# itz-sayak/C-Users-Sayakdutta-Self-Supervised-Arbitrary-Scale-Point-Cloud-Upsampling-via-SNN

Measured on AMD Instinct MI355X. Metric: upsampled query-points/sec (kNN + fn fwd + rotate + fd fwd + displace), 4x scale, M=48 T=4, higher is better.
Workload: dtype f32 (GEMMs as 3 x f16 MFMA with f32 accumulation; outer kNN f64); 1 GPU; synthetic sphere N=5000 (seed 0), B=4096 grid queries per GPU per step, M=48, T=4, fn k=[24,18,12] emb 640, fd k=32 scales [8,16,32,48] emb 768, conditioned-random weights seed 0, in-patch kNN recomputed every batch; cloud_points=5000, neighbours=48, outer_knn=f64 brute force, parallelism=query shards x1

## Files before the change

c-users-sayakdutta-self-supervised-arbitrary-scale-point-cloud-upsampling-via-snn_amd/_lib.py:

```python
import ctypes
import os
from ctypes import POINTER, c_char_p, c_double, c_float, c_int, c_int32, c_int64, c_void_p

_HERE = os.path.dirname(os.path.abspath(__file__))
LIB_PATH = os.environ.get("SAPCU_LIB_PATH") or os.path.join(_HERE, "csrc", "libsapcu_hip.so")
EXACT_LIB_PATH = os.path.join(_HERE, "csrc", "libsapcu_hip_exact.so")

FN_TAPS = ("stem", "block1", "block2", "block3", "pooled", "enc", "logits")
FD_TAPS = ("fused0", "spikes", "knn", "pooled", "enc", "x0")
KIND_FN, KIND_FD = 0, 1
ABI_VERSION = 2


class SapcuLibraryError(RuntimeError):
    """The HIP library is absent or unloadable (never silently replaced by a CPU path)."""


class SapcuError(RuntimeError):
    """A C entry point returned a non-zero status: args = (code, text)."""


_SIGNATURES = {
    "sapcu_abi_version": (c_int, []),
    "sapcu_last_error": (c_char_p, []),
# ... 64 lines not shown
_FD_TRAIN_SIGNATURES = {
    "sapcu_fd_neuron_step_forward": (c_int, [c_void_p, c_int64, c_int, c_int] + [c_void_p] * 6 + [c_void_p] * 3 + [c_void_p] + [c_void_p] * 5 +
                                     [c_void_p]),
    "sapcu_fd_neuron_step_workspace_bytes": (c_int64, [c_int64, c_int]),
    "sapcu_fd_neuron_step_backward": (c_int, [c_void_p, c_void_p, c_int64, c_int, c_int] + [c_void_p] * 4 + [c_void_p] * 3 + [c_void_p] * 5 +
                                      [c_void_p, c_int64, c_void_p]),
    "sapcu_fd_edge_feature_forward": (c_int, [c_void_p, c_int, c_void_p, c_int64, c_int, c_int, c_int, c_int, c_void_p, c_void_p, c_void_p]),
    "sapcu_fd_edge_feature_backward": (c_int, [c_void_p, c_void_p, c_int64, c_int, c_int, c_int, c_int, c_void_p, c_int, c_void_p, c_void_p]),
    "sapcu_fd_bn_stats_workspace_bytes": (c_int64, [c_int64, c_int]),
    "sapcu_fd_bn_stats": (c_int, [c_void_p, c_int64, c_int, c_float, c_void_p, c_void_p, c_void_p, c_void_p, c_int64, c_void_p]),
    "sapcu_fd_bn_lrelu_max_forward": (c_int, [c_void_p, c_int64, c_int, c_int] + [c_void_p] * 4 + [c_void_p, c_void_p, c_void_p]),
    "sapcu_fd_bn_lrelu_max_backward": (c_int, [c_void_p, c_void_p, c_void_p, c_int64, c_int, c_int] + [c_void_p] * 4 + [c_void_p, c_void_p]),
}
FD_TRAIN_EXPORTS = tuple(_FD_TRAIN_SIGNATURES)

_FD_EDGECONV_SIGNATURES = {
    "sapcu_fd_edgeconv_stats_workspace_bytes": (c_int64, [c_int64, c_int, c_int, c_int]),
    "sapcu_fd_edgeconv_stats": (c_int, [c_void_p, c_void_p, c_int64, c_int, c_int, c_int, c_float] + [c_void_p] * 4 + [c_void_p, c_int64, c_void_p]),
    "sapcu_fd_edgeconv_max_forward": (c_int, [c_void_p, c_void_p, c_int64, c_int, c_int, c_int] + [c_void_p] * 4 + [c_void_p, c_void_p, c_void_p]),
    "sapcu_fd_edgeconv_backward_workspace_bytes": (c_int64, [c_int64, c_int, c_int, c_int]),
    "sapcu_fd_edgeconv_backward": (c_int, [c_void_p] * 4 + [c_int64, c_int, c_int, c_int] + [c_void_p] * 4 + [c_void_p] * 4 +
                                   [c_void_p, c_int64, c_void_p]),
}
FD_EDGECONV_EXPORTS = tuple(_FD_EDGECONV_SIGNATURES)

_TRAIN_STEP_SIGNATURES = {
    "sapcu_multi_select": (c_int, [c_void_p, c_void_p, c_void_p, c_void_p, c_int, c_int, c_void_p]),
}
TRAIN_STEP_EXPORTS = tuple(_TRAIN_STEP_SIGNATURES)

_METRICS_SIGNATURES = {
    "sapcu_nn_cross_workspace_bytes": (c_int64, [c_int64, c_int64]),
    "sapcu_nn_cross_grid_f64": (c_int, [c_void_p, c_int64, c_void_p, c_int64, c_double, c_void_p, c_void_p, c_void_p, c_int64,
                                        POINTER(c_int64), c_void_p]),
}
METRICS_EXPORTS = tuple(_METRICS_SIGNATURES)

_DATA_SIGNATURES = {
    "sapcu_train_patches_workspace_bytes": (c_int64, [c_int64]),
    "sapcu_train_patches_f32": (c_int, [c_void_p, c_int64, c_int, c_void_p, c_int, c_void_p, c_void_p, c_int64, c_void_p, c_void_p, c_void_p,
                                        c_void_p, c_int, c_int] + [c_void_p] * 7 + [c_void_p, c_int64, c_void_p]),
}
DATA_EXPORTS = tuple(_DATA_SIGNATURES)

_MESH_SIGNATURES = {
    "sapcu_point_mesh_workspace_bytes": (c_int64, [c_int64, c_int64, c_int64]),
    "sapcu_point_mesh_f64": (c_int, [c_void_p, c_int64, c_void_p, c_int64, c_void_p, c_int64, c_double, c_void_p, c_void_p, c_void_p,
                                     c_void_p, c_int64, POINTER(c_int64), c_void_p]),
}
MESH_EXPORTS = tuple(_MESH_SIGNATURES)

_INTERNAL_SIGNATURES = {
    "sapcu_internal_fold_affine_host": (c_int, [c_void_p, c_void_p, c_void_p, c_void_p, c_int, c_int, c_void_p, c_void_p]),
    "sapcu_internal_point_mesh_tuned": (c_int, [c_void_p, c_int64, c_void_p, c_int64, c_void_p, c_int64, c_double, c_double, c_int, c_int, c_void_p,
                                                c_void_p, c_void_p, c_void_p, c_int64, POINTER(c_int64), c_void_p]),
}
_lib = None


def load(path=None):
    global _lib
    if _lib is not None and path is None:
        return _lib
    p = path or LIB_PATH
    if not os.path.exists(p):
        raise SapcuLibraryError(
            "HIP library not built: %s is missing. Run `make -C %s` (needs hipcc, gfx950). "
            "There is no CPU fallback." % (p, os.path.dirname(p)))
    try:
        lib = ctypes.CDLL(p)
    except OSError as e:
        raise SapcuLibraryError("cannot load %s: %s" % (p, e)) from e
    for name, (res, args) in list(_SIGNATURES.items()) + list(_SEEDS_SIGNATURES.items()) + list(_FD_TRAIN_SIGNATURES.items()) + \
            list(_FD_EDGECONV_SIGNATURES.items()) + list(_TRAIN_STEP_SIGNATURES.items()) + list(_METRICS_SIGNATURES.items()) + \
            list(_DATA_SIGNATURES.items()) + list(_MESH_SIGNATURES.items()) + list(_INTERNAL_SIGNATURES.items()):
        try:
            fn = getattr(lib, name)
        except AttributeError as e:
            raise SapcuLibraryError("%s does not export %s" % (p, name)) from e
        fn.restype = res
        fn.argtypes = args
    if lib.sapcu_abi_version() != ABI_VERSION:
        raise SapcuLibraryError("ABI version mismatch: library %d, binding %d" % (lib.sapcu_abi_version(), ABI_VERSION))
    if path is None:
        _lib = lib
    return lib


def check(rc):
    if rc != 0:
        text = load().sapcu_last_error()
        raise SapcuError(int(rc), text.decode("utf-8", "replace") if text else "")


def ptr(t):
    return None if t is None else c_void_p(t.data_ptr())


def current_stream():
    import torch
    return c_void_p(torch.cuda.current_stream().cuda_stream)
```

c-users-sayakdutta-self-supervised-arbitrary-scale-point-cloud-upsampling-via-snn_amd/csrc/common.h:

```cpp
#pragma once
#include <hip/hip_runtime.h>
#include <stdint.h>
#include <stdio.h>
#include <string.h>
#include "../../include/sapcu.h"

namespace sapcu {

void set_error(const char* fmt, ...);

#define SAPCU_CHECK_ARG(cond, ...)                      \
    do {                                                \
        if (!(cond)) {                                  \
            ::sapcu::set_error(__VA_ARGS__);            \
            return SAPCU_ERR_ARG;                       \
        }                                               \
    } while (0)

#define SAPCU_CHECK_HIP(expr)                                                            \
    do {                                                                                 \
        hipError_t _e = (expr);                                                          \
        if (_e != hipSuccess) {                                                          \
            ::sapcu::set_error("%s failed: %s (%s:%d)", #expr, hipGetErrorString(_e),    \
                               __FILE__, __LINE__);                                      \
// ... 382 lines not shown
    const double s = sqrt(d);
    const double r = __fma_rn(-s, s, d);
    return __fma_rn(r, __ddiv_rn(0.5, s), s);
}

__device__ __forceinline__ float gelu_erf(float x) {
    return 0.5f * x * (1.0f + erff(x * 0.70710678118654752440f));
}
__device__ __forceinline__ float lrelu02(float x) { return x >= 0.f ? x : 0.2f * x; }
__device__ __forceinline__ unsigned float_max_key(float x) {
    const unsigned b = __float_as_uint(x);
    return (b & 0x80000000u) ? ~b : (b | 0x80000000u);
}
__device__ __forceinline__ float float_from_max_key(unsigned k) { return __uint_as_float((k & 0x80000000u) ? (k & 0x7fffffffu) : ~k); }

enum GemmEpi { EPI_BIAS = 0, EPI_LIF = 1, EPI_GELU = 2, EPI_RESID = 3, EPI_LRELU = 4, EPI_RESID_GELU = 5, EPI_LIF_ATTN = 6,
               EPI_LRELU_MAX = 7,
               EPI_LIF_MAX = 8 };

struct GemmArgs {
    const float* a;
    int64_t r;
    int k, lda;
    const float* w;
    int n;
    const float* bias;
    float* c;
    int ldc;
    int epi;
    const float* lif;
    int lif_T;
    const float* resid;
    int ldr;
    float* c2;
    const float* q;
    const float* kf;
    int ldq;
    const int2* tab;
    const _Float16* w16_hi;
    const _Float16* w16_lo;
    int* ovf;
    int a_split, c_split, c2_split;
    unsigned* max_keys;
    int max_m;
    float* max_out;
};
int launch_gemm(const GemmArgs& g, hipStream_t st);
int launch_gemm_sf16(const GemmArgs& g, hipStream_t st);
int launch_gemm_sf16_ring(const GemmArgs& g, hipStream_t st);
int launch_gemm_sf16_bt(const GemmArgs& g, hipStream_t st);
bool gemm_sf16_bt_ok(const GemmArgs& g);
bool gemm_shortk_ok(const GemmArgs& g);
int launch_gemm_shortk(const GemmArgs& g, hipStream_t st);
int launch_gemm_split_rows(const GemmArgs& g, hipStream_t st, bool allow_bt = true);
int launch_split_weights(const float* w, int64_t count, void* hi, void* lo, int* ovf, hipStream_t st);

int launch_knn_outer(const double* cloud, int64_t n, const double* q, int64_t b, int k, int64_t* idx,
                     double* dist, float* patch, hipStream_t st);
int launch_gather_rotate(const double* cloud, int64_t n, const double* q, int64_t b, const int64_t* idx,
                         int k, const float* normals, float* patch, hipStream_t st);
int launch_displace(const double* q, const float* nrm, const float* d, int64_t b, double* out, hipStream_t st);

size_t fps_workspace_bytes(int npoint);
int zero_count(int* p, hipStream_t st);
int launch_fps(const float* xyz, int64_t n, int npoint, int start, int64_t* out, void* ws, hipStream_t st);
int fps_failed(const void* ws, int npoint, int* flag);

}
```

c-users-sayakdutta-self-supervised-arbitrary-scale-point-cloud-upsampling-via-snn_amd/csrc/gemm_epi.h:

```cpp
#pragma once
#include "common.h"

namespace sapcu {

typedef float f32x16 __attribute__((ext_vector_type(16)));

typedef _Float16 epi_half8 __attribute__((ext_vector_type(8)));
typedef float epi_f32x4 __attribute__((ext_vector_type(4)));
__device__ __forceinline__ f32x16 mfma_32x32x16_f16(epi_half8 a, epi_half8 b, f32x16 c) {
#ifdef SAPCU_TIMING_MFMA16
    epi_f32x4 q0 = {c[0], c[1], c[2], c[3]}, q1 = {c[8], c[9], c[10], c[11]};
    q0 = __builtin_amdgcn_mfma_f32_16x16x32_f16(a, b, q0, 0, 0, 0);
    q1 = __builtin_amdgcn_mfma_f32_16x16x32_f16(a, b, q1, 0, 0, 0);
    c[0] = q0[0]; c[1] = q0[1]; c[2] = q0[2]; c[3] = q0[3];
    c[8] = q1[0]; c[9] = q1[1]; c[10] = q1[2]; c[11] = q1[3];
    return c;
#else
    return __builtin_amdgcn_mfma_f32_32x32x16_f16(a, b, c, 0, 0, 0);
#endif
}

__device__ __forceinline__ float4 ld4(const float* p) { return *reinterpret_cast<const float4*>(p); }

__device__ __forceinline__ void lds_barrier() { asm volatile("s_waitcnt lgkmcnt(0)\n\ts_barrier" ::: "memory"); }
// ... 98 lines not shown
    if (EPI == EPI_LIF || EPI == EPI_LIF_ATTN) {
        const int cc = valid ? col : 0;
        c.decay = ld4_cols<VEC>(g.lif, cc, g.n);
        c.adapt = ld4_cols<VEC>(g.lif + g.n, cc, g.n);
        c.rdecay = ld4_cols<VEC>(g.lif + 2 * (int64_t)g.n, cc, g.n);
        c.theta0 = ld4_cols<VEC>(g.lif + 3 * (int64_t)g.n, cc, g.n);
    }
    return c;
}

__device__ __forceinline__ void clamp_col_params4(const ColParams4& c, NeuronP2 (&np)[2]) {
    np[0].decay = f32x2{clampf(c.decay.x, 0.1f, 0.99f), clampf(c.decay.y, 0.1f, 0.99f)};
    np[1].decay = f32x2{clampf(c.decay.z, 0.1f, 0.99f), clampf(c.decay.w, 0.1f, 0.99f)};
    np[0].adapt = f32x2{clampf(c.adapt.x, 0.001f, 0.1f), clampf(c.adapt.y, 0.001f, 0.1f)};
    np[1].adapt = f32x2{clampf(c.adapt.z, 0.001f, 0.1f), clampf(c.adapt.w, 0.001f, 0.1f)};
    np[0].rdecay = f32x2{clampf(c.rdecay.x, 0.1f, 0.95f), clampf(c.rdecay.y, 0.1f, 0.95f)};
    np[1].rdecay = f32x2{clampf(c.rdecay.z, 0.1f, 0.95f), clampf(c.rdecay.w, 0.1f, 0.95f)};
    np[0].theta0 = f32x2{c.theta0.x, c.theta0.y};
    np[1].theta0 = f32x2{c.theta0.z, c.theta0.w};
}

typedef _Float16 half4 __attribute__((ext_vector_type(4)));

template <bool VEC>
__device__ __forceinline__ void store_f32x4(float* base, int64_t row, int ld, int col, int n, const float (&v)[4]) {
    if (VEC) {
        *reinterpret_cast<float4*>(base + row * ld + col) = make_float4(v[0], v[1], v[2], v[3]);
    } else {
#pragma unroll
        for (int u = 0; u < 4; ++u)
            if (col + u < n) base[row * ld + col + u] = v[u];
    }
}

template <bool VEC>
__device__ __forceinline__ void store_split4(float* base, int64_t row, int ld, int col, int n, const float (&v)[4]) {
    if (!VEC) {
#pragma unroll
        for (int u = 0; u < 4; ++u)
            if (col + u < n) store_split(base, row, ld, col + u, v[u]);
        return;
    }
    _Float16* rp = reinterpret_cast<_Float16*>(base + row * ld);
    half4 hi, lo;
#pragma unroll
    for (int u = 0; u < 4; ++u) {
        hi[u] = (_Float16)v[u];
        lo[u] = (_Float16)(v[u] - (float)hi[u]);
    }
    *reinterpret_cast<half4*>(rp + split_hi_index(ld, col)) = hi;
    *reinterpret_cast<half4*>(rp + split_lo_index(ld, col)) = lo;
}

template <int EPI, bool VEC>
__device__ __forceinline__ void epilogue_row4_compute(const GemmArgs& g, const float4 acc, int64_t row, int col,
                                                      const ColParams4& cp, float (&v)[4]) {
    v[0] = __fmaf_rn(acc.x, 0.0625f, cp.bias.x);
    v[1] = __fmaf_rn(acc.y, 0.0625f, cp.bias.y);
    v[2] = __fmaf_rn(acc.z, 0.0625f, cp.bias.z);
    v[3] = __fmaf_rn(acc.w, 0.0625f, cp.bias.w);
    float4 res = make_float4(0.f, 0.f, 0.f, 0.f);
    if (EPI == EPI_RESID || EPI == EPI_RESID_GELU) res = ld4_cols<VEC>(g.resid + row * g.ldr, col, g.n);
    if (EPI == EPI_LIF || EPI == EPI_LIF_ATTN) {
        f32x2 pv[2] = {f32x2{v[0], v[1]}, f32x2{v[2], v[3]}};
        NeuronP2 np[2];
        clamp_col_params4(cp, np);
        lif_selfloop_pairs<2>(pv, np, g.lif_T);
        v[0] = pv[0].x; v[1] = pv[0].y; v[2] = pv[1].x; v[3] = pv[1].y;
    }
    const float rs[4] = {res.x, res.y, res.z, res.w};
#pragma unroll
    for (int u = 0; u < 4; ++u) {
        if (EPI == EPI_GELU) v[u] = gelu_erf(v[u]);
        if (EPI == EPI_LRELU) v[u] = lrelu02(v[u]);
        if (EPI == EPI_RESID) v[u] = __fadd_rn(v[u], rs[u]);
        if (EPI == EPI_RESID_GELU) v[u] = gelu_erf(__fadd_rn(v[u], rs[u]));
    }
}

template <int EPI, bool VEC>
__device__ __forceinline__ void epilogue_row4_store(const GemmArgs& g, const float (&v)[4], int64_t row, int col,
                                                    const float4 q, const float4 kf) {
    float ai[4] = {0.f, 0.f, 0.f, 0.f};
    if (EPI == EPI_LIF_ATTN) {
        ai[0] = __fadd_rn(__fsub_rn(q.x, kf.x), v[0]);
        ai[1] = __fadd_rn(__fsub_rn(q.y, kf.y), v[1]);
        ai[2] = __fadd_rn(__fsub_rn(q.z, kf.z), v[2]);
        ai[3] = __fadd_rn(__fsub_rn(q.w, kf.w), v[3]);
        asm volatile("" : "+v"(ai[0]), "+v"(ai[1]), "+v"(ai[2]), "+v"(ai[3])::"memory");
    }
    if (g.c_split) {
        store_split4<VEC>(g.c, row, g.ldc, col, g.n, v);
        if (EPI != EPI_LIF && EPI != EPI_LIF_ATTN && g.ovf) {
            float big = 0.f;
#pragma unroll
            for (int u = 0; u < 4; ++u)
                if (VEC || col + u < g.n) big = fmaxf(big, fabsf(v[u]));
            const bool nan = (VEC || col < g.n) && !(v[0] == v[0] && v[1] == v[1] && v[2] == v[2] && v[3] == v[3]);
            if (!(big < 65504.0f) || nan) atomicAdd(g.ovf, 1);
        }
    } else {
        store_f32x4<VEC>(g.c, row, g.ldc, col, g.n, v);
    }
    if (EPI == EPI_LIF_ATTN) {
        if (g.c2_split) store_split4<VEC>(g.c2, row, g.ldc, col, g.n, ai);
        else store_f32x4<VEC>(g.c2, row, g.ldc, col, g.n, ai);
    }
}

template <int EPI>
__device__ __forceinline__ void epilogue_group4(const GemmArgs& g, const float (&acc)[4], int64_t row, int col,
                                                float bias, const NeuronP& np, const float (&q)[4],
                                                const float (&kf)[4]) {
    epilogue_group<EPI, 4>(g, acc, row, col, bias, np, q, kf);
}

}
```

c-users-sayakdutta-self-supervised-arbitrary-scale-point-cloud-upsampling-via-snn_amd/csrc/model.hip:

```cpp
#include <stdarg.h>
#include <stdlib.h>

#include <new>
#include <vector>

#include "common.h"
#include "ops.h"

namespace sapcu {

static thread_local char g_err[512] = "";

void set_error(const char* fmt, ...) {
    va_list ap;
    va_start(ap, fmt);
    vsnprintf(g_err, sizeof(g_err), fmt, ap);
    va_end(ap);
}

enum FnSlot {
    FN_STEM_W = 0, FN_STEM_B, FN_STEM_LIF,
    FN_BLK0 = 3,
    FN_FINAL_W = FN_BLK0 + 63, FN_FINAL_B, FN_FINAL_LIF,
    FN_FCOUT_W, FN_FCOUT_B,
// ... 5 lines not shown
    B_FC1_W = 0, B_FC1_B, B_SNN1,
    B_QKV_W, B_QKV_B, B_QKV_LIF,
    B_DELTA_W, B_DELTA_B, B_DELTA_LIF,
    B_DELTA2_W, B_DELTA2_B, B_DELTA2_LIF,
    B_GAMMA_W, B_GAMMA_B, B_GAMMA_LIF,
    B_GAMMA2_W, B_GAMMA2_B,
    B_OUT_W, B_OUT_B,
    B_FC2_W, B_FC2_B,
    B_SLOTS
};
static_assert(B_SLOTS == 21, "fn block slot count");
static_assert(FN_SLOTS == 81, "fn slot count");

enum FdSlot {
    FD_E0_W = 0, FD_E0_B,
    FD_FUSE_W, FD_FUSE_B, FD_SNN0,
    FD_EDGE1_W, FD_EDGE1_SHIFT, FD_SNN1,
    FD_EDGE2_W, FD_EDGE2_SHIFT, FD_SNN2,
    FD_EDGE3_W, FD_EDGE3_SHIFT, FD_SNN3,
    FD_MSC_W, FD_MSC_B,
    FD_TI_W, FD_SNNFC,
    FD_FCIN_W, FD_FCIN_B,
    FD_R0_FC0_W, FD_R0_FC0_B, FD_R0_FC4_W, FD_R0_FC4_B, FD_R0_PROJ_W, FD_R0_PROJ_B,
    FD_R1_FC0_W, FD_R1_FC0_B, FD_R1_FC4_W, FD_R1_FC4_B, FD_R1_PROJ_W, FD_R1_PROJ_B,
    FD_QKV_W, FD_QKV_B,
    FD_WO_T, FD_BO, FD_LN_W, FD_LN_B, FD_WH_T, FD_BH, FD_WD, FD_BD,
    FD_SLOTS
};
static_assert(FD_SLOTS == 42, "fd slot count");

}

struct sapcu_model {
    int kind = 0;
    int kv[3] = {0, 0, 0};
    int k = 0, nscale = 0;
    int ks[8] = {0, 0, 0, 0, 0, 0, 0, 0};
    int32_t* ks_dev = nullptr;
    int* gate_dev = nullptr;
    bool sf16 = true;
    void* w16_hi = nullptr;
    void* w16_lo = nullptr;
    void* chain_w = nullptr;
    int* ovf_dev = nullptr;
    int emb = 0, T = 0, heads = 0;
    int64_t chunk = 0;
    int64_t ws_budget = 0;
    bool opt_bt = true;
    bool opt_chain = true;
    bool opt_chain_wide = false;
    bool opt_chain_fill = true;
    bool opt_chain_trim = true;
    bool opt_shortk = true;
    bool opt_fn_maxfuse = true;
    bool opt_fn_fold_out = true;
    bool opt_fd_maxfuse = true;
    bool opt_fd_split = true;
    bool opt_fd_fused = true;
    bool opt_fd_x0 = true;
    void* fde_w = nullptr;
    int64_t fde_off[5] = {0, 0, 0, 0, 0};
    float* fde_nprm = nullptr;
    float* blob = nullptr;
    int64_t blob_floats = 0;
    int64_t fold_w[3] = {0, 0, 0}, fold_b[3] = {0, 0, 0};
    std::vector<int64_t> dir;
    const float* p(int slot) const { return blob + dir[slot]; }
};

namespace sapcu {

static inline int64_t imax(int64_t a, int64_t b) { return a > b ? a : b; }
static inline int imin(int a, int b) { return a < b ? a : b; }

static bool split_rows_gemm_on_big_tile(const GemmArgs& g, bool allow_bt) { return allow_bt && gemm_sf16_bt_ok(g); }

int launch_gemm_split_rows(const GemmArgs& g, hipStream_t st, bool allow_bt) {
    if (split_rows_gemm_on_big_tile(g, allow_bt)) return launch_gemm_sf16_bt(g, st);
    return launch_gemm_sf16_ring(g, st);
}

static void fold_affine_f64(const float* w1, const float* b1, const float* w2, const float* b2, int d, int n, float* w_fold,
                            float* b_fold) {
    std::vector<double> acc((size_t)d);
    for (int i = 0; i < n; ++i) {
        for (int k = 0; k < d; ++k) acc[k] = 0.0;
        double bs = 0.0;
        for (int j = 0; j < d; ++j) {
            const double a = (double)w2[(int64_t)i * d + j];
            const float* row = w1 + (int64_t)j * d;
            for (int k = 0; k < d; ++k) acc[k] += a * (double)row[k];
            bs += a * (double)b1[j];
        }
        for (int k = 0; k < d; ++k) w_fold[(int64_t)i * d + k] = (float)acc[k];
        b_fold[i] = (float)(bs + (double)b2[i]);
    }
}

static bool env_is(const char* name, const char* value) {
    const char* e = getenv(name);
    return e && strcmp(e, value) == 0;
}

static void read_env_switches(sapcu_model* m) {
    m->sf16 = !env_is("SAPCU_GEMM", "f32");
    m->opt_bt = !env_is("SAPCU_BT", "0");
    m->opt_chain = !env_is("SAPCU_CHAIN", "0");
    m->opt_chain_wide = env_is("SAPCU_CHAIN", "wide");
    m->opt_chain_fill = !env_is("SAPCU_CHAIN_FILL", "0");
    m->opt_chain_trim = !env_is("SAPCU_CHAIN_TRIM", "0");
    m->opt_shortk = !env_is("SAPCU_SHORTK", "0");
    m->opt_fn_maxfuse = !env_is("SAPCU_FN_MAXFUSE", "0");
    m->opt_fn_fold_out = !env_is("SAPCU_FN_FOLD_OUT", "0");
    m->opt_fd_maxfuse = !env_is("SAPCU_FD_MAXFUSE", "0");
    m->opt_fd_split = !env_is("SAPCU_FD_SPLIT", "0");
    m->opt_fd_fused = !env_is("SAPCU_FD_FUSED", "0");
    m->opt_fd_x0 = !env_is("SAPCU_FD_X0", "0");
    const char* ce = getenv("SAPCU_CHUNK");
    m->chunk = ce ? atoll(ce) : 0;
    if (m->chunk < 0) m->chunk = 0;
    const char* be = getenv("SAPCU_WS_BUDGET_MB");
    m->ws_budget = (be ? atoll(be) : 20480) * (int64_t)(1 << 20);
    if (m->ws_budget < (int64_t)(64 << 20)) m->ws_budget = (int64_t)(64 << 20);
}

static void free_model(sapcu_model* m) {
    void* const owned[] = {m->w16_hi, m->w16_lo, m->chain_w, m->ovf_dev, m->blob, m->ks_dev, m->gate_dev, m->fde_w, m->fde_nprm};
    for (void* p : owned)
        if (p) (void)hipFree(p);
    delete m;
}

static int run_gemm(const sapcu_model* m, GemmArgs& g, hipStream_t st) {
    const bool have16 = m && m->sf16 && g.w >= m->blob && g.w < m->blob + m->blob_floats;
    if (have16) {
        const int64_t off = g.w - m->blob;
        g.w16_hi = (const _Float16*)m->w16_hi + off;
        g.w16_lo = (const _Float16*)m->w16_lo + off;
        g.ovf = m->ovf_dev;
        if (g.a_split) return launch_gemm_split_rows(g, st, m->opt_bt);
        if (m->opt_shortk && gemm_shortk_ok(g)) return launch_gemm_shortk(g, st);
        if (g.max_out) {
            set_error("run_gemm: a direct max output needs the short-K kernel");
            return SAPCU_ERR_ARG;
        }
        if (g.k % 64 == 0) return launch_gemm_sf16(g, st);
    }
    if (g.a_split || g.c_split || g.c2_split) {
        set_error("run_gemm: split-row operands need the split-f16 kernels");
        return SAPCU_ERR_ARG;
    }
    return launch_gemm(g, st);
}

static int gemm(const sapcu_model* m, const float* a, int64_t r, int k, int lda, const float* w, int n,
                const float* bias, float* c, int ldc, int epi, hipStream_t st, const float* lif = nullptr,
                int lifT = 0, const float* resid = nullptr, int ldr = 0, int fmt = 0) {
    GemmArgs g;
    memset(&g, 0, sizeof(g));
    g.a = a; g.r = r; g.k = k; g.lda = lda; g.w = w; g.n = n; g.bias = bias; g.c = c; g.ldc = ldc;
    g.epi = epi; g.lif = lif; g.lif_T = lifT; g.resid = resid; g.ldr = ldr;
    g.a_split = fmt & 1; g.c_split = (fmt >> 1) & 1;
    return run_gemm(m, g, st);
}

#define SAPCU_TRY(expr)                 \
    do {                                \
        int _rc = (expr);               \
        if (_rc != SAPCU_OK) return _rc; \
    } while (0)

static int tap_copy(void* const* taps, int which, int64_t dst_off_bytes, const void* src, int64_t bytes,
                    hipStream_t st) {
    if (!taps || !taps[which] || bytes == 0) return SAPCU_OK;
    SAPCU_CHECK_HIP(hipMemcpyAsync((char*)taps[which] + dst_off_bytes, src, (size_t)bytes, hipMemcpyDeviceToDevice, st));
    return SAPCU_OK;
}

struct FnPlan {
    int64_t cb;
    int kk[3], kmx;
    int64_t edge_floats, edge_floats23;
};

static bool fn_block_fused(const sapcu_model* m, int l, int mp) {
    return m->sf16 && m->chain_w && m->opt_chain && fn_edge_chain_ok(128 << l, imin(m->kv[l], mp));
}

static int fn_kmax(const sapcu_model* m, int mp) {
    int kmx = 1;
    for (int l = 0; l < 3; ++l) kmx = kmx > imin(m->kv[l], mp) ? kmx : imin(m->kv[l], mp);
    return kmx;
}
// ... 550 lines not shown
                                  threshold_base, delta_T, theta_rh, spikes_out, membrane_out, threshold_out,
                                  refractory_out, (hipStream_t)stream);
}

int sapcu_neuron_drive(const float* x, int64_t rows, int channels, int steps, const float* membrane_decay,
                       const float* threshold_adapt, const float* refractory_decay, const float* threshold_base,
                       const float* delta_T, const float* theta_rh, int channel_pairs, float* spikes_out, float* membrane_out,
                       float* threshold_out, float* refractory_out, int* gate_open_out, void* stream) {
    SAPCU_CHECK_ARG(x && membrane_decay && threshold_adapt && refractory_decay && threshold_base, "neuron_drive: null pointer");
    SAPCU_CHECK_ARG((delta_T == nullptr) == (theta_rh == nullptr), "neuron_drive: delta_T and theta_rh go together");
    SAPCU_CHECK_ARG(rows >= 0 && channels >= 1 && steps >= 1, "neuron_drive: bad sizes");
    return launch_neuron_drive(x, rows, channels, steps, membrane_decay, threshold_adapt, refractory_decay, threshold_base, delta_T,
                               theta_rh, channel_pairs, spikes_out, membrane_out, threshold_out, refractory_out, gate_open_out,
                               (hipStream_t)stream);
}

int sapcu_patch_knn(const float* feat, int64_t b, int m, int c, int ld, int k, int32_t* idx_out, void* stream) {
    SAPCU_CHECK_ARG(feat && idx_out && b >= 0 && ld >= c, "patch_knn: bad argument");
    return launch_patch_knn(feat, b, m, c, ld, k, idx_out, (hipStream_t)stream);
}

int sapcu_l2_normalize3(const float* in, float* out, int64_t b, void* stream) {
    SAPCU_CHECK_ARG(in && out && b >= 0, "l2_normalize3: bad argument");
    return launch_l2_normalize3(in, out, b, (hipStream_t)stream);
}

static int split_into_ws(const float* w, int64_t cnt, void* w16_ws, GemmArgs& g, hipStream_t st) {
    char* base = (char*)w16_ws;
    int* ovf = (int*)(base + 4 * cnt);
    SAPCU_CHECK_HIP(hipMemsetAsync(ovf, 0, sizeof(int), st));
    SAPCU_TRY(launch_split_weights(w, cnt, base, base + 2 * cnt, ovf, st));
    g.w16_hi = (const _Float16*)base;
    g.w16_lo = (const _Float16*)(base + 2 * cnt);
    g.ovf = ovf;
    return SAPCU_OK;
}

int sapcu_gemm_f32(const float* a, int64_t r, int k, int lda, const float* w, int n, const float* bias,
                   const float* lif4, int lif_steps, float* c, int ldc, void* w16_ws, int a_split_rows, int c_split_rows,
                   void* stream) {
    SAPCU_CHECK_ARG(a && w && c && r >= 0 && n >= 1, "gemm: bad argument");
    SAPCU_CHECK_ARG(!lif4 || lif_steps >= 1, "gemm: lif_steps must be >= 1");
    SAPCU_CHECK_ARG(!(a_split_rows || c_split_rows) || w16_ws, "gemm: split rows need the split-f16 kernels (w16_ws)");
    SAPCU_CHECK_ARG(r == 0 || (k > 0 && k % 32 == 0 && lda >= k && ldc >= n), "gemm: need k %% 32 == 0, lda >= k and ldc >= n (k=%d lda=%d n=%d ldc=%d)", k, lda, n, ldc);
    SAPCU_CHECK_ARG(r == 0 || ((((uintptr_t)a | (uintptr_t)w | (uintptr_t)w16_ws) & 15) == 0 && lda % (a_split_rows ? 8 : 4) == 0),
                    "gemm: A, W and w16_ws must be 16-byte aligned, lda %% 4 == 0 (%% 8 for split rows) (lda=%d)", lda);
    GemmArgs g;
    memset(&g, 0, sizeof(g));
    g.a = a; g.r = r; g.k = k; g.lda = lda; g.w = w; g.n = n; g.bias = bias; g.c = c; g.ldc = ldc;
    g.epi = lif4 ? EPI_LIF : EPI_BIAS; g.lif = lif4; g.lif_T = lif_steps;
    g.a_split = a_split_rows ? 1 : 0; g.c_split = c_split_rows ? 1 : 0;
    if (w16_ws && (g.a_split || k % 64 == 0)) {
        SAPCU_TRY(split_into_ws(w, (int64_t)n * k, w16_ws, g, (hipStream_t)stream));
        if (g.a_split) return launch_gemm_split_rows(g, (hipStream_t)stream, a_split_rows != 2);
        if (!env_is("SAPCU_SHORTK", "0") && gemm_shortk_ok(g)) return launch_gemm_shortk(g, (hipStream_t)stream);
        return launch_gemm_sf16(g, (hipStream_t)stream);
    }
    SAPCU_CHECK_ARG(!g.c_split, "gemm: split-row output needs k %% 64 == 0 on the f32-A path");
    return launch_gemm(g, (hipStream_t)stream);
}

int sapcu_to_split_rows(const float* in, int64_t rows, int k, int ld_in, float* out, int ld_out, void* stream) {
    SAPCU_CHECK_ARG(in && out && rows >= 0 && k >= 1 && ld_in >= k && ld_out >= k, "to_split_rows: bad argument");
    return launch_to_split_rows(in, rows, k, ld_in, out, ld_out, (hipStream_t)stream);
}

int sapcu_posenc_gemm_f32(const float* pe1, int64_t r, int d, const float* w, const float* bias, const float* lif4,
                          int lif_steps, const float* qkv, const int32_t* idx, int kk, int m_pts, float* pe_out,
                          float* attn_in_out, void* edge_table_ws, void* w16_ws, int split_rows, void* stream) {
    SAPCU_CHECK_ARG(pe1 && w && lif4 && qkv && idx && pe_out && attn_in_out && edge_table_ws && r >= 0 && d >= 32 &&
                        lif_steps >= 1 && kk >= 1 && m_pts >= 1,
                    "posenc_gemm: bad argument");
    SAPCU_CHECK_ARG(!split_rows || w16_ws, "posenc_gemm: split rows need the split-f16 kernels (w16_ws)");
    SAPCU_CHECK_ARG(d % 32 == 0, "posenc_gemm: d=%d must be a multiple of 32", d);
    SAPCU_CHECK_ARG((((uintptr_t)pe1 | (uintptr_t)w | (uintptr_t)w16_ws) & 15) == 0 && ((uintptr_t)edge_table_ws & 7) == 0,
                    "posenc_gemm: pe1, w and w16_ws must be 16-byte aligned, edge_table_ws 8-byte aligned");
    GemmArgs g;
    memset(&g, 0, sizeof(g));
    g.a = pe1; g.r = r; g.k = d; g.lda = d; g.w = w; g.n = d; g.bias = bias; g.c = pe_out; g.ldc = d;
    g.epi = EPI_LIF_ATTN; g.lif = lif4; g.lif_T = lif_steps; g.c2 = attn_in_out;
    g.q = qkv; g.kf = qkv + d; g.ldq = 3 * d; g.tab = (const int2*)edge_table_ws;
    SAPCU_TRY(launch_edge_table(idx, r, m_pts, kk, (int2*)edge_table_ws, (hipStream_t)stream));
    if (w16_ws && (split_rows || d % 64 == 0)) {
        SAPCU_TRY(split_into_ws(w, (int64_t)d * d, w16_ws, g, (hipStream_t)stream));
        if (split_rows) {
            g.a_split = 1;
            g.c2_split = 1;
            return launch_gemm_split_rows(g, (hipStream_t)stream, split_rows != 2);
        }
        return launch_gemm_sf16(g, (hipStream_t)stream);
    }
    return launch_gemm(g, (hipStream_t)stream);
}

struct ChainWs {
    int2* tab;
    float4* pd;
    char* split[3];
    _Float16* packed[3];
    size_t bytes;
};

static ChainWs chain_ws_layout(void* base, int64_t points, int d, int kk) {
    WsCarver c(base);
    ChainWs w;
    w.tab = c.take<int2>(points * kk);
    w.pd = c.take<float4>(points * kk);
// ... 173 lines not shown
                        const int64_t wo = m->dir[FN_BLK0 + l * B_SLOTS + slots[q]];
                        if (launch_pack_chain_weights((const _Float16*)m->w16_hi + wo, (const _Float16*)m->w16_lo + wo, d,
                                                      (_Float16*)m->chain_w + chain_w_off(l, q), nullptr) != SAPCU_OK)
                            rc = SAPCU_ERR_HIP;
                    }
                }
                if (rc == SAPCU_OK) hip_ok(hipDeviceSynchronize(), "pack chain weights");
            }
        }
        if (rc == SAPCU_OK && kind == SAPCU_KIND_FD) {
            hip_ok(hipMalloc((void**)&m->ks_dev, 8 * sizeof(int32_t)), "hipMalloc(ks)");
            if (rc == SAPCU_OK) hip_ok(hipMemcpy(m->ks_dev, m->ks, 8 * sizeof(int32_t), hipMemcpyHostToDevice), "copy ks");
            if (rc == SAPCU_OK) hip_ok(hipMalloc((void**)&m->gate_dev, sizeof(int)), "hipMalloc(gate)");
            if (rc == SAPCU_OK) hip_ok(hipMemset(m->gate_dev, 0, sizeof(int)), "memset gate");
            if (rc == SAPCU_OK && m->sf16 && m->emb >= 96) {
                const int first = m->nscale <= 4 ? 0 : 4;
                const int mats[5][3] = {{FD_FUSE_W, 64, 64 * m->nscale}, {FD_EDGE1_W, 256, 64}, {FD_EDGE2_W, 512, 128},
                                        {FD_EDGE3_W, 1024, 256}, {FD_MSC_W, m->emb, 960}};
                int64_t halves = 0;
                for (int i = 0; i < 5; ++i) {
                    m->fde_off[i] = halves;
                    if (i >= first) halves += (int64_t)2 * mats[i][1] * mats[i][2];
                }
                hip_ok(hipMalloc(&m->fde_w, (size_t)halves * 2), "hipMalloc(fde_w)");
                if (rc == SAPCU_OK) hip_ok(hipMalloc((void**)&m->fde_nprm, 960 * 8 * sizeof(float)), "hipMalloc(fde_nprm)");
                for (int i = first; i < 5 && rc == SAPCU_OK; ++i) {
                    const int64_t wo = m->dir[mats[i][0]];
                    if (launch_pack_frag_weights((const _Float16*)m->w16_hi + wo, (const _Float16*)m->w16_lo + wo, mats[i][1], mats[i][2],
                                                 (_Float16*)m->fde_w + m->fde_off[i], nullptr) != SAPCU_OK)
                        rc = SAPCU_ERR_HIP;
                }
                static const int nslot[4] = {FD_SNN0, FD_SNN1, FD_SNN2, FD_SNN3}, nch[4] = {64, 128, 256, 512}, noff[4] = {0, 64, 192, 448};
                for (int i = 0; i < 4 && rc == SAPCU_OK; ++i)
                    if (launch_pack_fd_neuron(m->p(nslot[i]), nch[i], i < 2 ? 1 : 0, noff[i], m->fde_nprm, nullptr) != SAPCU_OK) rc = SAPCU_ERR_HIP;
                if (rc == SAPCU_OK) hip_ok(hipDeviceSynchronize(), "pack fd encoder operands");
            }
        }
    }
    if (rc != SAPCU_OK) {
        free_model(m);
        return rc;
    }
    *out = m;
    return SAPCU_OK;
}

int sapcu_internal_fold_affine_host(const float* w_out, const float* b_out, const float* w_fc2, const float* b_fc2, int d, int n,
                                    float* w_fold_out, float* b_fold_out) {
    SAPCU_CHECK_ARG(w_out && b_out && w_fc2 && b_fc2 && w_fold_out && b_fold_out && d >= 1 && n >= 1, "fold_affine: bad argument");
    fold_affine_f64(w_out, b_out, w_fc2, b_fc2, d, n, w_fold_out, b_fold_out);
    return SAPCU_OK;
}

int sapcu_model_destroy(sapcu_model_t m) {
    if (!m) return SAPCU_OK;
    free_model(m);
    return SAPCU_OK;
}

int64_t sapcu_workspace_bytes(sapcu_model_t m, int64_t b, int m_pts) {
    if (!m || b < 0 || m_pts < 1 || m_pts > 128) {
        set_error("workspace_bytes: bad argument");
        return SAPCU_ERR_ARG;
    }
    const size_t bytes = m->kind == SAPCU_KIND_FN ? fn_ws_layout(nullptr, m, fn_plan(m, b, m_pts), m_pts).bytes
                                                  : fd_ws_layout(nullptr, m, fd_plan(m, b, m_pts), m_pts).bytes;
    return (int64_t)bytes + 256;
}

int sapcu_model_gate_violations(sapcu_model_t m, int* count_host) {
    SAPCU_CHECK_ARG(m && count_host, "gate_violations: null pointer");
    *count_host = 0;
    if (m->gate_dev) SAPCU_CHECK_HIP(hipMemcpy(count_host, m->gate_dev, sizeof(int), hipMemcpyDeviceToHost));
    return SAPCU_OK;
}

int sapcu_model_gemm_mode(sapcu_model_t m, int* split_f16_host, int* range_overflows_host) {
    SAPCU_CHECK_ARG(m && split_f16_host && range_overflows_host, "gemm_mode: null pointer");
    *split_f16_host = m->sf16 ? 1 : 0;
    *range_overflows_host = 0;
    if (m->ovf_dev) SAPCU_CHECK_HIP(hipMemcpy(range_overflows_host, m->ovf_dev, sizeof(int), hipMemcpyDeviceToHost));
    return SAPCU_OK;
}

int sapcu_model_fused_blocks(sapcu_model_t m, int m_pts, int* mask_host) {
    SAPCU_CHECK_ARG(m && mask_host && m_pts >= 1 && m_pts <= 128, "fused_blocks: bad argument");
    int mask = 0;
    if (m->kind == SAPCU_KIND_FN) {
        for (int l = 0; l < 3; ++l)
            if (fn_block_fused(m, l, m_pts)) mask |= 1 << l;
    } else {
        if (fd_encoder_fused(m, m_pts)) mask = 1;
        else if (fd_x0_path(m, m_pts)) mask = 2;
    }
    *mask_host = mask;
    return SAPCU_OK;
}

int sapcu_fn_forward(sapcu_model_t m, const float* patch, int64_t b, int m_pts, const int32_t* knn_in, int32_t* knn_out,
                     float* normals_out, void* workspace, int64_t ws_bytes, void* const* taps_host, void* stream) {
    SAPCU_CHECK_ARG(m && m->kind == SAPCU_KIND_FN, "fn_forward: not an fn model handle");
    SAPCU_CHECK_ARG(patch && normals_out && workspace, "fn_forward: null pointer");
    SAPCU_CHECK_ARG(b >= 0 && m_pts >= 1 && m_pts <= 128, "fn_forward: need 1 <= m_pts <= 128 (got %d)", m_pts);
    return fn_forward(m, patch, b, m_pts, knn_in, knn_out, normals_out, workspace, ws_bytes, taps_host,
                      (hipStream_t)stream);
}
// ... 11 lines not shown
```

Measured before the change: 134,000 query-points/s.

## Add narrow-N split-f16 GEMM kernel with LDS-resident weights for n=64

Adds a dedicated GEMM kernel for split-row inputs with exactly 64 output columns and K up to 512. The whole hi/lo f16 weight tile is loaded into LDS once per block with global_load_lds. Each wave then walks a persistent stream of 32-row blocks, prefetching its A fragments in registers D steps ahead. The bias/residual epilogue is refactored so the residual can be loaded early and passed in. This targets narrow layers where the general big-tile or ring kernels waste tile width and reload weights; the risk is the extra LDS per block and the loss of the old kernel's tuning for these shapes.

```diff
diff --git a/c-users-sayakdutta-self-supervised-arbitrary-scale-point-cloud-upsampling-via-snn_amd/_lib.py b/c-users-sayakdutta-self-supervised-arbitrary-scale-point-cloud-upsampling-via-snn_amd/_lib.py
--- a/c-users-sayakdutta-self-supervised-arbitrary-scale-point-cloud-upsampling-via-snn_amd/_lib.py
+++ b/c-users-sayakdutta-self-supervised-arbitrary-scale-point-cloud-upsampling-via-snn_amd/_lib.py
@@ -140,6 +140,7 @@
 
 _INTERNAL_SIGNATURES = {
     "sapcu_internal_fold_affine_host": (c_int, [c_void_p, c_void_p, c_void_p, c_void_p, c_int, c_int, c_void_p, c_void_p]),
+    "sapcu_internal_gemm_narrow_serves": (c_int, [c_int, c_int, c_int]),
     "sapcu_internal_point_mesh_tuned": (c_int, [c_void_p, c_int64, c_void_p, c_int64, c_void_p, c_int64, c_double, c_double, c_int, c_int, c_void_p,
                                                 c_void_p, c_void_p, c_void_p, c_int64, POINTER(c_int64), c_void_p]),
 }
diff --git a/c-users-sayakdutta-self-supervised-arbitrary-scale-point-cloud-upsampling-via-snn_amd/csrc/common.h b/c-users-sayakdutta-self-supervised-arbitrary-scale-point-cloud-upsampling-via-snn_amd/csrc/common.h
--- a/c-users-sayakdutta-self-supervised-arbitrary-scale-point-cloud-upsampling-via-snn_amd/csrc/common.h
+++ b/c-users-sayakdutta-self-supervised-arbitrary-scale-point-cloud-upsampling-via-snn_amd/csrc/common.h
@@ -458,7 +458,10 @@
 bool gemm_sf16_bt_ok(const GemmArgs& g);
 bool gemm_shortk_ok(const GemmArgs& g);
 int launch_gemm_shortk(const GemmArgs& g, hipStream_t st);
-int launch_gemm_split_rows(const GemmArgs& g, hipStream_t st, bool allow_bt = true);
+bool gemm_narrow_shape_ok(int n, int k, int epi);
+bool gemm_narrow_ok(const GemmArgs& g);
+int launch_gemm_narrow(const GemmArgs& g, hipStream_t st);
+int launch_gemm_split_rows(const GemmArgs& g, hipStream_t st, bool allow_bt = true, bool allow_narrow = true);
 int launch_split_weights(const float* w, int64_t count, void* hi, void* lo, int* ovf, hipStream_t st);
 
 int launch_knn_outer(const double* cloud, int64_t n, const double* q, int64_t b, int k, int64_t* idx,
diff --git a/c-users-sayakdutta-self-supervised-arbitrary-scale-point-cloud-upsampling-via-snn_amd/csrc/gemm_epi.h b/c-users-sayakdutta-self-supervised-arbitrary-scale-point-cloud-upsampling-via-snn_amd/csrc/gemm_epi.h
--- a/c-users-sayakdutta-self-supervised-arbitrary-scale-point-cloud-upsampling-via-snn_amd/csrc/gemm_epi.h
+++ b/c-users-sayakdutta-self-supervised-arbitrary-scale-point-cloud-upsampling-via-snn_amd/csrc/gemm_epi.h
@@ -174,15 +174,13 @@
     *reinterpret_cast<half4*>(rp + split_lo_index(ld, col)) = lo;
 }
 
-template <int EPI, bool VEC>
-__device__ __forceinline__ void epilogue_row4_compute(const GemmArgs& g, const float4 acc, int64_t row, int col,
-                                                      const ColParams4& cp, float (&v)[4]) {
+template <int EPI>
+__device__ __forceinline__ void epilogue_row4_compute_res(const GemmArgs& g, const float4 acc, const ColParams4& cp, const float4 res,
+                                                          float (&v)[4]) {
     v[0] = __fmaf_rn(acc.x, 0.0625f, cp.bias.x);
     v[1] = __fmaf_rn(acc.y, 0.0625f, cp.bias.y);
     v[2] = __fmaf_rn(acc.z, 0.0625f, cp.bias.z);
     v[3] = __fmaf_rn(acc.w, 0.0625f, cp.bias.w);
-    float4 res = make_float4(0.f, 0.f, 0.f, 0.f);
-    if (EPI == EPI_RESID || EPI == EPI_RESID_GELU) res = ld4_cols<VEC>(g.resid + row * g.ldr, col, g.n);
     if (EPI == EPI_LIF || EPI == EPI_LIF_ATTN) {
         f32x2 pv[2] = {f32x2{v[0], v[1]}, f32x2{v[2], v[3]}};
         NeuronP2 np[2];
@@ -198,6 +196,14 @@
         if (EPI == EPI_RESID) v[u] = __fadd_rn(v[u], rs[u]);
         if (EPI == EPI_RESID_GELU) v[u] = gelu_erf(__fadd_rn(v[u], rs[u]));
     }
+}
+
+template <int EPI, bool VEC>
+__device__ __forceinline__ void epilogue_row4_compute(const GemmArgs& g, const float4 acc, int64_t row, int col,
+                                                      const ColParams4& cp, float (&v)[4]) {
+    float4 res = make_float4(0.f, 0.f, 0.f, 0.f);
+    if (EPI == EPI_RESID || EPI == EPI_RESID_GELU) res = ld4_cols<VEC>(g.resid + row * g.ldr, col, g.n);
+    epilogue_row4_compute_res<EPI>(g, acc, cp, res, v);
 }
 
 template <int EPI, bool VEC>
diff --git a/c-users-sayakdutta-self-supervised-arbitrary-scale-point-cloud-upsampling-via-snn_amd/csrc/gemm_narrow.hip b/c-users-sayakdutta-self-supervised-arbitrary-scale-point-cloud-upsampling-via-snn_amd/csrc/gemm_narrow.hip
--- /dev/null
+++ b/c-users-sayakdutta-self-supervised-arbitrary-scale-point-cloud-upsampling-via-snn_amd/csrc/gemm_narrow.hip
@@ -0,0 +1,220 @@
+#include "common.h"
+#include "gemm_epi.h"
+
+namespace sapcu {
+
+typedef _Float16 nhalf8 __attribute__((ext_vector_type(8)));
+
+constexpr int NBM = 32;
+constexpr int NBN = 64;
+constexpr int NBK = 32;
+constexpr int NWAVES = 8;
+constexpr int NKMAX = 512;
+constexpr int NWPLANE = NBN * NBK * 2;
+constexpr int NWSTEP = 2 * NWPLANE;
+constexpr int NHAND = NBM * 32 * 4;
+static inline int narrow_lds_bytes(int k) { return (k / NBK) * NWSTEP + NWAVES * NHAND; }
+
+struct NarrowA {
+    nhalf8 h0, h1, l0, l1;
+};
+
+typedef __attribute__((address_space(3))) unsigned char nlds_byte;
+typedef const __attribute__((address_space(1))) void* ngptr_t;
+
+__device__ __forceinline__ nhalf8 a_load8(const char* p) { return *reinterpret_cast<const nhalf8*>(p); }
+
+template <int EPI, int D>
+__global__ __launch_bounds__(NWAVES * 64) void gemm_narrow_kernel(const GemmArgs g) {
+    extern __shared__ __attribute__((aligned(1024))) unsigned char smem_raw[];
+    const int tid = threadIdx.x;
+    const int lane = tid & 63;
+    const int wave = __builtin_amdgcn_readfirstlane(tid >> 6);
+    const int r32 = lane & 31, h = lane >> 5;
+    const int nk = g.k / NBK;
+    float* const hand = reinterpret_cast<float*>(smem_raw + nk * NWSTEP) + wave * (NHAND / 4);
+
+    const int64_t nb = (g.r + NBM - 1) / NBM;
+    const int64_t wtiles = nb > wave ? (nb - wave + NWAVES - 1) / NWAVES : 0;
+    const int64_t my_blocks = wtiles > (int64_t)blockIdx.x ? (wtiles - blockIdx.x + gridDim.x - 1) / gridDim.x : 0;
+    const int64_t blk_first = (int64_t)blockIdx.x * NWAVES + wave, blk_step = (int64_t)gridDim.x * NWAVES;
+
+    const bool a_il = (g.lda & 31) == 0;
+    const int kstep_bytes = a_il ? 128 : NBK * 2;
+    const int64_t lo_delta = a_il ? 64 : 2 * (int64_t)g.lda;
+    const int64_t pitch_b = 4 * (int64_t)g.lda;
+    const char* const a_base = reinterpret_cast<const char*>(g.a) + h * 16;
+    int64_t pf_blk = blk_first, pf_left = my_blocks * nk;
+    int pf_kt = 0;
+    const char* pf_row = a_base;
+    auto pf_setup = [&]() {
+        int64_t row = pf_blk * NBM + r32;
+        if (row >= g.r) row = g.r - 1;
+        pf_row = a_base + row * pitch_b;
+    };
+    auto issue = [&](NarrowA& f) {
+        const char* s = pf_row + pf_kt * kstep_bytes;
+        f.h0 = a_load8(s);
+        f.h1 = a_load8(s + 32);
+        f.l0 = a_load8(s + lo_delta);
+        f.l1 = a_load8(s + lo_delta + 32);
+        if (pf_left > 0) --pf_left;
+        if (++pf_kt == nk) {
+            pf_kt = 0;
+            if (pf_left > 0) {
+                pf_blk += blk_step;
+                pf_setup();
+            }
+        }
+    };
+    {
+        const int wrow = (wave & 3) * 16 + (lane >> 2);
+        const char* src = reinterpret_cast<const char*>((wave >> 2) ? g.w16_lo : g.w16_hi) + (int64_t)wrow * (2 * g.k) +
+                          (((lane & 3) ^ ((lane >> 4) & 3)) * 16);
+        nlds_byte* dst = (nlds_byte*)(smem_raw + (wave >> 2) * NWPLANE + (wave & 3) * 1024);
+        for (int kt = 0; kt < nk; ++kt) __builtin_amdgcn_global_load_lds((ngptr_t)(src + kt * (NBK * 2)), dst + kt * NWSTEP, 16, 0, 0);
+    }
+    asm volatile("" ::: "memory");
+    NarrowA buf[D];
+    if (pf_left) pf_setup();
+#pragma unroll
+    for (int j = 0; j < D; ++j) issue(buf[j]);
+    asm volatile("s_waitcnt vmcnt(%0)" ::"n"(4 * D) : "memory");
+    lds_barrier();
+
+    int woff[2][2];
+#pragma unroll
+    for (int j = 0; j < 2; ++j)
+#pragma unroll
+        for (int k16 = 0; k16 < 2; ++k16) {
+            const int wr = j * 32 + r32;
+            woff[j][k16] = wr * (NBK * 2) + (((k16 * 2 + h) ^ ((wr >> 2) & 3)) * 16);
+        }
+    const int c4 = lane & 7, rs = lane >> 3;
+    float* const hand_even = hand + 5 * h * 32 + r32;
+    float* const hand_odd = hand + 3 * h * 32 + r32;
+    ColParams4 cp[2];
+#pragma unroll
+    for (int j = 0; j < 2; ++j) {
+        cp[j].bias = cp[j].decay = cp[j].adapt = cp[j].rdecay = cp[j].theta0 = make_float4(0.f, 0.f, 0.f, 0.f);
+        if (g.bias) cp[j].bias = ld4(g.bias + j * 32 + c4 * 4);
+        settle4(cp[j].bias);
+    }
+
+    f32x16 acc[2];
+    auto step = [&](NarrowA& f, int kt) {
+        const unsigned char* sw = smem_raw + kt * NWSTEP;
+        nhalf8 wh[2][2], wl[2][2];
+#pragma unroll
+        for (int j = 0; j < 2; ++j)
+#pragma unroll
+            for (int k16 = 0; k16 < 2; ++k16) {
+                wh[j][k16] = *reinterpret_cast<const nhalf8*>(sw + woff[j][k16]);
+                wl[j][k16] = *reinterpret_cast<const nhalf8*>(sw + woff[j][k16] + NWPLANE);
+            }
+        acc[0] = mfma_32x32x16_f16(f.l0, wh[0][0], acc[0]);
+        acc[1] = mfma_32x32x16_f16(f.l0, wh[1][0], acc[1]);
+        acc[0] = mfma_32x32x16_f16(f.l1, wh[0][1], acc[0]);
+        acc[1] = mfma_32x32x16_f16(f.l1, wh[1][1], acc[1]);
+        acc[0] = mfma_32x32x16_f16(f.h0, wl[0][0], acc[0]);
+        acc[1] = mfma_32x32x16_f16(f.h0, wl[1][0], acc[1]);
+        acc[0] = mfma_32x32x16_f16(f.h1, wl[0][1], acc[0]);
+        acc[1] = mfma_32x32x16_f16(f.h1, wl[1][1], acc[1]);
+        acc[0] = mfma_32x32x16_f16(f.h0, wh[0][0], acc[0]);
+        acc[1] = mfma_32x32x16_f16(f.h0, wh[1][0], acc[1]);
+        acc[0] = mfma_32x32x16_f16(f.h1, wh[0][1], acc[0]);
+        acc[1] = mfma_32x32x16_f16(f.h1, wh[1][1], acc[1]);
+        issue(f);
+    };
+
+    int64_t blk = blk_first;
+    for (int64_t bi = 0; bi < my_blocks; ++bi, blk += blk_step) {
+#pragma unroll
+        for (int j = 0; j < 2; ++j)
+#pragma unroll
+            for (int e = 0; e < 16; ++e) acc[j][e] = 0.f;
+        int kt = 0;
+        for (; kt < nk - D; kt += D) {
+#pragma unroll
+            for (int b = 0; b < D; ++b) step(buf[b], kt + b);
+        }
+        float4 res[2][4];
+#pragma unroll
+        for (int j = 0; j < 2; ++j)
+#pragma unroll
+            for (int p = 0; p < 4; ++p) {
+                res[j][p] = make_float4(0.f, 0.f, 0.f, 0.f);
+                if (EPI == EPI_RESID) {
+                    int64_t row = blk * NBM + p * 8 + rs;
+                    if (row >= g.r) row = g.r - 1;
+                    res[j][p] = ld4(g.resid + row * g.ldr + j * 32 + c4 * 4);
+                }
+            }
+#pragma unroll
+        for (int b = 0; b < D; ++b) step(buf[b], kt + b);
+#pragma unroll
+        for (int j = 0; j < 2; ++j) {
+#pragma unroll
+            for (int e = 0; e < 16; ++e) {
+                float* hb = (e & 1) ? hand_odd : hand_even;
+                hb[((e & 3) + 8 * (e >> 2)) * 32] = acc[j][e];
+            }
+            asm volatile("s_waitcnt lgkmcnt(0)" ::: "memory");
+#pragma unroll
+            for (int p = 0; p < 4; ++p) {
+                const int rr = p * 8 + rs;
+                const int64_t row = blk * NBM + rr;
+                const int col = j * 32 + c4 * 4;
+                const float4 a = *reinterpret_cast<const float4*>(hand + (rr ^ ((rr >> 2) & 1)) * 32 + c4 * 4);
+                if (EPI == EPI_RESID) settle4(res[j][p]);
+                if (row >= g.r) continue;
+                float v[4];
+                epilogue_row4_compute_res<EPI>(g, a, cp[j], res[j][p], v);
+                const float4 z = make_float4(0.f, 0.f, 0.f, 0.f);
+                epilogue_row4_store<EPI, true>(g, v, row, col, z, z);
+            }
+            asm volatile("s_waitcnt lgkmcnt(0)" ::: "memory");
+        }
+    }
+}
+
+bool gemm_narrow_shape_ok(int n, int k, int epi) {
+    return n == NBN && k >= NBK && k % NBK == 0 && k <= NKMAX && (epi == EPI_BIAS || epi == EPI_RESID);
+}
+
+bool gemm_narrow_ok(const GemmArgs& g) {
+    auto al16 = [](const void* p) { return ((uintptr_t)p & 15) == 0; };
+    if (!g.a_split || !g.w16_hi || !g.w16_lo || !gemm_narrow_shape_ok(g.n, g.k, g.epi)) return false;
+    if (g.k > g.lda || g.lda % 8 || !al16(g.a) || !al16(g.w16_hi) || !al16(g.w16_lo)) return false;
+    if (g.ldc % 4 || g.ldc < NBN || !al16(g.c) || (g.bias && !al16(g.bias))) return false;
+    if (g.epi == EPI_RESID && (!g.resid || g.ldr % 4 || g.ldr < NBN || !al16(g.resid))) return false;
+    return true;
+}
+
+template <int EPI, int D>
+static int launch_narrow_td(const GemmArgs& g, hipStream_t st) {
+    static DeviceOnce lds_once;
+    SAPCU_SET_MAX_LDS(lds_once, (&gemm_narrow_kernel<EPI, D>), narrow_lds_bytes(NKMAX));
+    const int64_t wtiles = ((g.r + NBM - 1) / NBM + NWAVES - 1) / NWAVES;
+    const int cus = device_cu_count();
+    const int64_t grid = wtiles < cus ? wtiles : cus;
+    hipLaunchKernelGGL((gemm_narrow_kernel<EPI, D>), dim3((unsigned)grid), dim3(NWAVES * 64), narrow_lds_bytes(g.k), st, g);
+    SAPCU_CHECK_LAUNCH();
+    return SAPCU_OK;
+}
+
+template <int EPI>
+static int launch_narrow_t(const GemmArgs& g, hipStream_t st) {
+    const int nk = g.k / NBK;
+    if (nk % 4 == 0) return launch_narrow_td<EPI, 4>(g, st);
+    if (nk % 2 == 0) return launch_narrow_td<EPI, 2>(g, st);
+    return launch_narrow_td<EPI, 1>(g, st);
+}
+
+int launch_gemm_narrow(const GemmArgs& g, hipStream_t st) {
+    if (g.r == 0) return SAPCU_OK;
+    SAPCU_CHECK_ARG(gemm_narrow_ok(g), "gemm_narrow: shape, epilogue or alignment not served (n=%d k=%d epi=%d)", g.n, g.k, g.epi);
+    return g.epi == EPI_RESID ? launch_narrow_t<EPI_RESID>(g, st) : launch_narrow_t<EPI_BIAS>(g, st);
+}
+
+}
diff --git a/c-users-sayakdutta-self-supervised-arbitrary-scale-point-cloud-upsampling-via-snn_amd/csrc/model.hip b/c-users-sayakdutta-self-supervised-arbitrary-scale-point-cloud-upsampling-via-snn_amd/csrc/model.hip
--- a/c-users-sayakdutta-self-supervised-arbitrary-scale-point-cloud-upsampling-via-snn_amd/csrc/model.hip
+++ b/c-users-sayakdutta-self-supervised-arbitrary-scale-point-cloud-upsampling-via-snn_amd/csrc/model.hip
@@ -81,6 +81,7 @@
     bool opt_chain_fill = true;
     bool opt_chain_trim = true;
     bool opt_shortk = true;
+    bool opt_narrown = true;
     bool opt_fn_maxfuse = true;
     bool opt_fn_fold_out = true;
     bool opt_fd_maxfuse = true;
@@ -104,7 +105,8 @@
 
 static bool split_rows_gemm_on_big_tile(const GemmArgs& g, bool allow_bt) { return allow_bt && gemm_sf16_bt_ok(g); }
 
-int launch_gemm_split_rows(const GemmArgs& g, hipStream_t st, bool allow_bt) {
+int launch_gemm_split_rows(const GemmArgs& g, hipStream_t st, bool allow_bt, bool allow_narrow) {
+    if (allow_narrow && gemm_narrow_ok(g)) return launch_gemm_narrow(g, st);
     if (split_rows_gemm_on_big_tile(g, allow_bt)) return launch_gemm_sf16_bt(g, st);
     return launch_gemm_sf16_ring(g, st);
 }
@@ -139,6 +141,7 @@
     m->opt_chain_fill = !env_is("SAPCU_CHAIN_FILL", "0");
     m->opt_chain_trim = !env_is("SAPCU_CHAIN_TRIM", "0");
     m->opt_shortk = !env_is("SAPCU_SHORTK", "0");
+    m->opt_narrown = !env_is("SAPCU_NARROWN", "0");
     m->opt_fn_maxfuse = !env_is("SAPCU_FN_MAXFUSE", "0");
     m->opt_fn_fold_out = !env_is("SAPCU_FN_FOLD_OUT", "0");
     m->opt_fd_maxfuse = !env_is("SAPCU_FD_MAXFUSE", "0");
@@ -167,7 +170,7 @@
         g.w16_hi = (const _Float16*)m->w16_hi + off;
         g.w16_lo = (const _Float16*)m->w16_lo + off;
         g.ovf = m->ovf_dev;
-        if (g.a_split) return launch_gemm_split_rows(g, st, m->opt_bt);
+        if (g.a_split) return launch_gemm_split_rows(g, st, m->opt_bt, m->opt_narrown);
         if (m->opt_shortk && gemm_shortk_ok(g)) return launch_gemm_shortk(g, st);
         if (g.max_out) {
             set_error("run_gemm: a direct max output needs the short-K kernel");
@@ -824,7 +827,8 @@
     g.a_split = a_split_rows ? 1 : 0; g.c_split = c_split_rows ? 1 : 0;
     if (w16_ws && (g.a_split || k % 64 == 0)) {
         SAPCU_TRY(split_into_ws(w, (int64_t)n * k, w16_ws, g, (hipStream_t)stream));
-        if (g.a_split) return launch_gemm_split_rows(g, (hipStream_t)stream, a_split_rows != 2);
+        if (g.a_split)
+            return launch_gemm_split_rows(g, (hipStream_t)stream, a_split_rows != 2, a_split_rows != 2 && !env_is("SAPCU_NARROWN", "0"));
         if (!env_is("SAPCU_SHORTK", "0") && gemm_shortk_ok(g)) return launch_gemm_shortk(g, (hipStream_t)stream);
         return launch_gemm_sf16(g, (hipStream_t)stream);
     }
@@ -1104,6 +1108,10 @@
     return SAPCU_OK;
 }
 
+int sapcu_internal_gemm_narrow_serves(int n, int k, int with_residual) {
+    return gemm_narrow_shape_ok(n, k, with_residual ? EPI_RESID : EPI_BIAS) ? 1 : 0;
+}
+
 int sapcu_model_destroy(sapcu_model_t m) {
     if (!m) return SAPCU_OK;
     free_model(m);
```

New measurement: 134,300 query-points/s, median of 6. About the same (+0.2%).
